# vigorbird/ORB_SLAM2_comment

Hardware: AMD Instinct MI355X
Metric: frames/sec ORB extract+match, KITTI 1241×376 @1000 feat; HBM GB/s vs peak (higher is better)
Workload: dtype u8; 1 GPU; configs[1]+[2]+[3]: a global batch of 512 synthetic 1241x376 u8 frames per step, 512 per GPU, resident in HBM as (last, cur) pairs; per step ORB extract (nFeatures=1000, 8-level pyramid) of every frame + device-resident SearchByProjection(CurrentFrame, LastFrame, th=15, mono; projection prologue included) for every pair; monocular handles: mvImagePyramid[0] on demand (orbhip_extractor_set_lazy_lev; handles_per_gpu=3, stage_gates=0, global_batch=512, nfeatures=1000, levels=8, parallelism=pair-sharded x1

## Files before the change

orb_slam2_comment_amd/csrc/orbhip_matcher.hip:

```cpp
#include "orbhip_internal.h"

#include <algorithm>
#include <climits>
#include <new>
#include <vector>

namespace orbhip {

constexpr int TH_HIGH = 100, TH_LOW = 50, HISTO_LENGTH = 30;
constexpr int GRID_ROWS = 48, GRID_COLS = 64;
constexpr int kResolveMax = 4096;
constexpr uint32_t kNoCell = 0xffffffffu;

struct DevFrame {
    int n;
    const orbhip_keypoint *keys;
    const uint8_t *desc;
    const float *u_right;
    float min_x, min_y, inv_w, inv_h;
};

struct Batch {
    const int *n_dev;
    const int *nq_dev;
// ... 30 lines not shown
        const uint32_t lo_ = (uint32_t)v, hi_ = (uint32_t)(v >> 32);                                          \
        const uint32_t ol_ = (uint32_t)__builtin_amdgcn_update_dpp((int)lo_, (int)lo_, ctrl, rmask, 0xf, false); \
        const uint32_t oh_ = (uint32_t)__builtin_amdgcn_update_dpp((int)hi_, (int)hi_, ctrl, rmask, 0xf, false); \
        const unsigned long long o_ = ((unsigned long long)oh_ << 32) | ol_;                                  \
        v = o_ < v ? o_ : v;                                                                                  \
    }
    ORBHIP_MIN64_STEP(0xB1, 0xf)
    ORBHIP_MIN64_STEP(0x4E, 0xf)
    ORBHIP_MIN64_STEP(0x141, 0xf)
    ORBHIP_MIN64_STEP(0x140, 0xf)
    ORBHIP_MIN64_STEP(0x142, 0xa)
    ORBHIP_MIN64_STEP(0x143, 0xc)
#undef ORBHIP_MIN64_STEP
    return ((unsigned long long)(uint32_t)__builtin_amdgcn_readlane((int)(v >> 32), 63) << 32) |
           (uint32_t)__builtin_amdgcn_readlane((int)(uint32_t)v, 63);
}

constexpr int kHeadMax = 8;
__device__ __forceinline__ int wave_sorted_head(unsigned long long a1, unsigned long long a2, bool more,
                                                unsigned long long (&head)[kHeadMax], bool *complete)
{
    int given = 0, hl = 0;
    bool stop = false, dry = false;
#pragma unroll
    for (int k = 0; k < kHeadMax; ++k) {
        head[k] = ~0ull;
        if (stop || dry) continue;
        const unsigned long long c = given == 0 ? a1 : (given == 1 ? a2 : ~0ull);
        const unsigned long long g = wave_min_u64(c);
        if (g == ~0ull) { dry = true; continue; }
// ... 120 lines not shown

constexpr int kGridCells = GRID_COLS * GRID_ROWS;
struct GridRec { float x, y; int octave; uint32_t key; };
__device__ __forceinline__ void grid_build_body(DevFrame F, int *__restrict__ cell_start, GridRec *__restrict__ rec,
                                                uint4 *__restrict__ rdesc, float *__restrict__ rur, const Batch &B, const int pair)
{
    __shared__ int s_cnt[kGridCells];
    __shared__ int s_scan[8];
    const int tid = threadIdx.x;
    batch_frame(F, B, pair);
    const size_t rbase = (size_t)pair * B.cap;
    cell_start += (size_t)pair * (kGridCells + 1);
    rec += rbase; rdesc += rbase * 2; rur += rbase;
    for (int c = tid; c < kGridCells; c += 256) s_cnt[c] = 0;
    __syncthreads();
    for (int j = tid; j < F.n; j += 256) {
        const orbhip_keypoint kp = F.keys[j];
        const int px = (int)roundf(__fmul_rn(__fsub_rn(kp.x, F.min_x), F.inv_w));
        const int py = (int)roundf(__fmul_rn(__fsub_rn(kp.y, F.min_y), F.inv_h));
        if (!(px < 0 || px >= GRID_COLS || py < 0 || py >= GRID_ROWS)) atomicAdd(&s_cnt[px * GRID_ROWS + py], 1);
    }
    __syncthreads();
    constexpr int PER = kGridCells / 256;
    int local[PER], sum = 0;
#pragma unroll
    for (int k = 0; k < PER; ++k) { local[k] = s_cnt[tid * PER + k]; sum += local[k]; }
    int incl = sum;
    const int lane = tid & 63, wave = tid >> 6;
    incl = wave_incl_scan_add(incl);
    if (lane == 63) s_scan[wave] = incl;
    __syncthreads();
    int base = incl - sum;
    for (int w = 0; w < wave; ++w) base += s_scan[w];
    __syncthreads();
#pragma unroll
    for (int k = 0; k < PER; ++k) { s_cnt[tid * PER + k] = base; cell_start[tid * PER + k] = base; base += local[k]; }
    if (tid == 255) cell_start[kGridCells] = base;
    __syncthreads();
    for (int j = tid; j < F.n; j += 256) {
        const orbhip_keypoint kp = F.keys[j];
        const int px = (int)roundf(__fmul_rn(__fsub_rn(kp.x, F.min_x), F.inv_w));
        const int py = (int)roundf(__fmul_rn(__fsub_rn(kp.y, F.min_y), F.inv_h));
        if (!(px < 0 || px >= GRID_COLS || py < 0 || py >= GRID_ROWS)) {
            const int cell = px * GRID_ROWS + py;
            const int pos = atomicAdd(&s_cnt[cell], 1);
            GridRec r; r.x = kp.x; r.y = kp.y; r.octave = kp.octave; r.key = ((uint32_t)cell << 20) | (uint32_t)j;
            rec[pos] = r;
            const uint4 *d = reinterpret_cast<const uint4 *>(F.desc + (size_t)j * 32);
            rdesc[2 * pos] = d[0]; rdesc[2 * pos + 1] = d[1];
            rur[pos] = F.u_right ? F.u_right[j] : -1.0f;
        }
    }
}
__global__ __launch_bounds__(256) void k_grid_build(DevFrame F, int *__restrict__ cell_start, GridRec *__restrict__ rec,
                                                    uint4 *__restrict__ rdesc, float *__restrict__ rur, Batch B)
{
    grid_build_body(F, cell_start, rec, rdesc, rur, B, (int)blockIdx.x);
}

constexpr int kCompact = 64;
__global__ __launch_bounds__(256) void k_window_search(DevFrame F, const int *__restrict__ cell_start,
                                                       const GridRec *__restrict__ rec, const uint4 *__restrict__ rdesc,
                                                       const float *__restrict__ rur,
                                                       const orbhip_query *__restrict__ q,
                                                       const uint8_t *__restrict__ qdesc,
                                                       unsigned long long *__restrict__ cand,
                                                       unsigned long long *__restrict__ ccand,
                                                       int *__restrict__ cnt, int stride, int use_ur, Batch B,
                                                       const uint8_t *__restrict__ taken, int max_dist)
{
    __shared__ unsigned long long stage[4][64];
    __shared__ int spos[4][64];
    const int lane = threadIdx.x & 63, wv = threadIdx.x >> 6;
    const int pair = blockIdx.y;
    const bool has_ur = F.u_right != nullptr;
    batch_frame(F, B, pair);
// ... 845 lines not shown
    S.lcn = lcn;
    S.lc = reinterpret_cast<uint32_t *>(base + resolve_par_bytes(n, nq, 0));
    int *p = reinterpret_cast<int *>(base);
    S.owner[0] = p; p += n; S.owner[1] = p; p += n; S.choice = p; p += nq;
    S.t_angle = reinterpret_cast<float *>(p); p += n; S.q_angle = reinterpret_cast<float *>(p); p += nq;
    S.hist = p; p += HISTO_LENGTH + 2; S.vars = p; p += 16;
    S.cur1 = reinterpret_cast<unsigned short *>(p); S.cur2 = S.cur1 + nq; p += nq;
    S.wl[0] = reinterpret_cast<unsigned short *>(p); S.wl[1] = S.wl[0] + nq; p += nq;
    S.q_cnt = p; p += nq;
    unsigned char *c = reinterpret_cast<unsigned char *>(p);
    S.t_oct = c; c += n; S.taken = c; c += n; S.q_obs = c; c += nq; S.evbin = c;
}

#ifdef ORBHIP_DEVTOOLS
__device__ unsigned int g_resolve_stats[4];
#endif
template <bool GS>
__global__ __launch_bounds__(1024) void k_resolve_par(int mode, DevFrame F, const orbhip_query *__restrict__ q, int nq,
                                                      const unsigned long long *__restrict__ cand,
                                                      const unsigned long long *__restrict__ ccand,
                                                      const int *__restrict__ cnt, int stride,
                                                      const uint8_t *__restrict__ taken_in, float nnratio,
                                                      int check_ori, int *__restrict__ out, int *__restrict__ out_n, Batch B,
                                                      int th_accept, int all_block, unsigned char *__restrict__ gstate,
                                                      size_t gstate_stride, int lcn)
{
    extern __shared__ unsigned char resolve_lds[];
    const int tid = threadIdx.x, T = blockDim.x;
    {
        const int pair = blockIdx.x;
        batch_frame(F, B, pair);
        q += (size_t)pair * B.qcap;
        cand += (size_t)pair * B.qcap * stride;
        if (ccand) ccand += (size_t)pair * B.qcap * kCompact;
        cnt += (size_t)pair * B.qcap;
        if (taken_in) taken_in += (size_t)pair * B.cap;
        out += (size_t)pair * B.cap;
        out_n += pair;
        if (B.nq_dev) nq = min(B.nq_dev[pair], B.qcap);
    }
    const int n = F.n;
    ResolveParState S;
    if (GS) resolve_par_carve(S, gstate + (size_t)blockIdx.x * gstate_stride, (size_t)n, (size_t)nq);
// ... 42 lines not shown
                    S.lc[i * (S.lcn + 1) + S.lcn] = (uint32_t)hrow[kHeadMax];
                }
                continue;
            }
            if (i != tid || !ccand) {
                const unsigned long long *l0 = ccand ? ccand + (size_t)i * kCompact : cand + (size_t)i * stride;
#pragma unroll
                for (int e = 0; e < kResolveHead; ++e) hv[e] = (e < c && e < S.lcn) ? l0[e] : ~0ull;
            }
#pragma unroll
            for (int e = 0; e < kResolveHead; ++e)
                if (e < c && e < S.lcn) S.lc[i * (S.lcn + 1) + e] = ((uint32_t)(hv[e] >> 32) << 20) | (uint32_t)(hv[e] & 0xfffffu);
        }
    }
    __syncthreads();
    auto held_by_smaller = [&](int idx, int i) -> bool {
        return S.taken[idx] || __hip_atomic_load(&holder[idx], __ATOMIC_RELAXED, __HIP_MEMORY_SCOPE_WORKGROUP) < i;
    };
    unsigned short *wl_next = nullptr;
    int *wl_count = nullptr;
    int *claim = holder;
    bool claims_rebuilt = false;
    auto pick_sorted = [&](int i, int c, unsigned long long &k1, unsigned long long &k2) {
        const unsigned long long *list = ccand ? ccand + (size_t)i * kCompact : cand + (size_t)i * stride;
        const uint32_t *lrow = S.lc + i * (S.lcn + 1);
        auto entry = [&](int e) -> unsigned long long {
            if (e >= c) return ~0ull;
            if (!GS && e < S.lcn) { const uint32_t w = lrow[e]; return ((unsigned long long)(w >> 20) << 32) | (w & 0xfffffu); }
            return list[e];
        };
// ... 139 lines not shown
                const int src = __ffsll((long long)longs) - 1;
                unsigned long long t1, t2;
                pick_unsorted_wave(__builtin_amdgcn_readlane(i, src), -__builtin_amdgcn_readlane(c, src), t1, t2);
                if (lane == src) { k1 = t1; k2 = t2; }
                longs &= longs - 1;
            }
        }
        return valid && c != 0 ? commit(i, k1, k2) : (valid ? commit(i, ~0ull, ~0ull) : false);
    };
    if (mode != 1) {
        int c_in = 5, c_out = 6, c_clr = 7, rounds = 0;
        unsigned short *w_in = S.wl[0], *w_out = S.wl[1];
        wl_next = w_out; wl_count = &S.vars[c_out];
        for (int i0 = 0; i0 < nq; i0 += T) step_group(i0 + tid, i0 + tid < nq);
        __syncthreads();
        for (;; ++rounds) {
            { unsigned short *t_ = w_in; w_in = w_out; w_out = t_; }
            { const int t_ = c_in; c_in = c_out; c_out = c_clr; c_clr = t_; }
            const int nw = S.vars[c_in];
            if (nw == 0 || rounds > 65 * nq) break;
            if (tid == 0) S.vars[c_clr] = 0;
            wl_next = w_out; wl_count = &S.vars[c_out];
            for (int k0 = 0; k0 < nw; k0 += T) step_group(k0 + tid < nw ? (int)w_in[k0 + tid] : 0, k0 + tid < nw);
            __syncthreads();
        }
        wl_next = nullptr;
        bool unobs = false;
        for (int i = tid; i < nq; i += T) unobs |= !S.q_obs[i];
        if (__syncthreads_or(unobs))
            for (int i0 = 0; i0 < nq; i0 += T) step_group(i0 + tid, i0 + tid < nq && !S.q_obs[i0 + tid]);
#ifdef ORBHIP_DEVTOOLS
        if (tid == 0) { atomicAdd(&g_resolve_stats[0], 1u); atomicAdd(&g_resolve_stats[1], (unsigned)rounds + 1); atomicMax(&g_resolve_stats[2], (unsigned)rounds + 1); }
#endif
    } else {
        int *own_cur = S.owner[0], *own_nxt = S.owner[1];
        claims_rebuilt = true;
        for (int round = 0; round <= nq + 1; ++round) {
            if (tid == 0) S.vars[0] = 0;
            for (int c = tid; c < n; c += T) own_nxt[c] = INT_MAX;
            __syncthreads();
            holder = own_cur; claim = own_nxt;
// ... 1 lines not shown
            for (int i0 = 0; i0 < nq; i0 += T) ch |= step_group(i0 + tid, i0 + tid < nq);
            if (ch) S.vars[0] = 1;
            __syncthreads();
            const int changed = S.vars[0];
            { int *t_ = own_cur; own_cur = own_nxt; own_nxt = t_; }
            __syncthreads();
            if (!changed) {
#ifdef ORBHIP_DEVTOOLS
                if (tid == 0) { atomicAdd(&g_resolve_stats[0], 1u); atomicAdd(&g_resolve_stats[1], (unsigned)round + 1); atomicMax(&g_resolve_stats[2], (unsigned)round + 1); }
#endif
                break;
            }
        }
    }
    __syncthreads();
    int *assign = S.owner[1];
    for (int c = tid; c < n; c += T) assign[c] = -1;
    __syncthreads();
    int acc_local = 0;
    const bool ori = mode == 0 && check_ori;
    for (int i0 = 0; i0 < nq; i0 += T) {
        const int i = i0 + tid;
        const int c = i < nq ? S.choice[i] : -1;
        int bin = -1;
        if (c >= 0) {
            ++acc_local;
            atomicMax(&assign[c], i);
            if (ori) {
                bin = rot_bin(S.q_angle[i], S.t_angle[c]);
                if (bin >= 0) S.evbin[i] = (unsigned char)bin;
            }
        }
        wave_hist_add(S.hist, bin);
    }
    acc_local = wave_reduce_add_i(acc_local);
    if ((tid & 63) == 0 && acc_local) atomicAdd(&S.vars[1], acc_local);
    __syncthreads();
    if (ori) {
        rank_bins_once(S.hist, S.vars + 8);
        const int ind1 = S.vars[8], ind2 = S.vars[9], ind3 = S.vars[10];
        int cull = 0;
        for (int i = tid; i < nq; i += T) {
            if (rot_culled(S.evbin[i], ind1, ind2, ind3)) {
                assign[S.choice[i]] = -1;
                ++cull;
            }
        }
        cull = wave_reduce_add_i(cull);
        if ((tid & 63) == 0 && cull) atomicAdd(&S.vars[2], cull);
        __syncthreads();
    }
    for (int c = tid; c < n; c += T) out[c] = assign[c];
    if (tid == 0) *out_n = S.vars[1] - S.vars[2];
}

struct InitState {
    int *q_cnt; float *q_angle, *t_angle;
    uint32_t *claim[2];
    int *head[2];
    unsigned short *next[2];
    unsigned char *evbin;
    int *hist, *vars;
    unsigned short *active;
    unsigned short *active_u;
    uint32_t *lc; int lcn;
};
constexpr uint32_t kNoClaim = 0xffffffffu;
__host__ __device__ constexpr size_t init_state_bytes(size_t n, size_t nq, size_t lcn)
// ... 993 lines not shown
    const float *Tcw;
    const orbhip_keypoint *keys;
    const uint8_t *desc;
    const int *n_dev;
    const float *u_right;
    const int *cell_start, *cell_items;
    const float *world, *normal, *max_dist, *min_dist;
    const uint8_t *point_desc, *flags;
    int *best_idx, *best_dist;
    orbhip_query *q;
    int cap, np, pcap;
    int sim3_form;
    int csr_by_target;
    float min_x, min_y, inv_w, inv_h;
};

template <int LPQ> __device__ __forceinline__ unsigned long long group_min_u64(unsigned long long v);
template <> __device__ __forceinline__ unsigned long long group_min_u64<64>(unsigned long long v) { return wave_min_u64(v); }
template <> __device__ __forceinline__ unsigned long long group_min_u64<8>(unsigned long long v)
{
#define ORBHIP_GMIN_STEP(ctrl)                                                                                \
    {                                                                                                         \
        const uint32_t lo_ = (uint32_t)v, hi_ = (uint32_t)(v >> 32);                                          \
        const uint32_t ol_ = (uint32_t)__builtin_amdgcn_update_dpp((int)lo_, (int)lo_, ctrl, 0xf, 0xf, false); \
        const uint32_t oh_ = (uint32_t)__builtin_amdgcn_update_dpp((int)hi_, (int)hi_, ctrl, 0xf, 0xf, false); \
        const unsigned long long o_ = ((unsigned long long)oh_ << 32) | ol_;                                  \
        v = o_ < v ? o_ : v;                                                                                  \
    }
    ORBHIP_GMIN_STEP(0xB1)
    ORBHIP_GMIN_STEP(0x4E)
    ORBHIP_GMIN_STEP(0x141)
#undef ORBHIP_GMIN_STEP
    return v;
}

template <int LPQ>
__global__ __launch_bounds__(256) void k_fuse_batch(FuseBatchArgs A, orbhip_camera cam, float th, SigmaTab sig)
{
    const int k = blockIdx.y, lane = threadIdx.x & 63;
    const int i = blockIdx.x * 256 + threadIdx.x;
    const size_t f = (size_t)A.kf_index[k], orow = (size_t)k * A.pcap;
    orbhip_query Q;
    Q.valid = 0; Q.u = 0; Q.v = 0; Q.radius = 0; Q.min_level = 0; Q.ur = 0;
    if (i < A.np) {
        KfQueryArgs P;
        P.T1 = A.Tcw + (size_t)k * 12; P.T2 = nullptr;
        P.world = A.world; P.normal = A.normal; P.max_dist = A.max_dist; P.min_dist = A.min_dist;
        P.flags = A.flags + orow; P.q = nullptr; P.n = A.np; P.mode = 0; P.double_invz = A.sim3_form;
        Q = keyframe_query(P, cam, th, i);
// ... 544 lines not shown
    __syncthreads();
    if (tid < 2) counts[(size_t)f * 2 + tid] = s_cnt[tid];
}

}

using namespace orbhip;

struct orbhip_matcher {
    int device = 0;
    hipStream_t stream = nullptr;
    hipStream_t own_stream = nullptr;
    void *buf[17] = {};
    size_t cap[17] = {};
    bool lds_attr_set = false, bow_attr_set = false;
    uint8_t *h_stage = nullptr; size_t h_stage_bytes = 0;
    uint8_t *h_out = nullptr; size_t h_out_bytes = 0;
};

static inline size_t al256(size_t b) { return (b + 255) & ~(size_t)255; }

struct Stage {
    uint8_t *h, *d;
    size_t off, cap;
    bool overrun;
    template <class T> T *take(size_t count, const T **dev)
    {
        const size_t bytes = al256(count * sizeof(T));
        if (overrun || bytes > cap - off) { overrun = true; *dev = nullptr; return nullptr; }
        *dev = reinterpret_cast<const T *>(d + off);
// ... 64 lines not shown
        m->h_out_bytes = bytes;
    }
    ORBHIP_HIP_CHECK(hipMemcpyAsync(m->h_out, d, bytes, hipMemcpyDeviceToHost, m->stream));
    ORBHIP_HIP_CHECK(hipStreamSynchronize(m->stream));
    *h = m->h_out;
    return ORBHIP_OK;
}

static int ensure_resolve_attr(orbhip_matcher *m)
{
    if (!m->lds_attr_set) {
        ORBHIP_HIP_CHECK(hipFuncSetAttribute(reinterpret_cast<const void *>(k_resolve_par<false>), hipFuncAttributeMaxDynamicSharedMemorySize,
                                             kResolveLdsBudget));
        ORBHIP_HIP_CHECK(hipFuncSetAttribute(reinterpret_cast<const void *>(k_resolve_init), hipFuncAttributeMaxDynamicSharedMemorySize,
                                             kResolveLdsBudget));
        m->lds_attr_set = true;
    }
    return ORBHIP_OK;
}

static_assert(init_state_bytes(kResolveMax, kResolveMax, 0) <= (size_t)kResolveLdsBudget, "k_resolve_init state exceeds LDS");

static int launch_resolve_par(orbhip_matcher *m, int pairs, int mode, const DevFrame &D, const orbhip_query *d_q,
                              const unsigned long long *d_cand, const unsigned long long *d_ccand, const int *d_cnt, int stride,
                              const uint8_t *d_taken, float nnratio, int check_ori, int *d_out, int *d_out_n, const Batch &B,
                              int th_accept, int all_block)
{
    if (B.cap <= kResolveMax && B.qcap <= kResolveMax) {
        const int lcn = resolve_par_bytes((size_t)B.cap, (size_t)B.qcap, kResolveHead) <= (size_t)kResolveLdsBudget ? kResolveHead : 0;
        hipLaunchKernelGGL(k_resolve_par<false>, dim3(pairs), dim3(1024), resolve_par_bytes((size_t)B.cap, (size_t)B.qcap, (size_t)lcn),
                           m->stream, mode, D, d_q, B.qcap, d_cand, d_ccand, d_cnt, stride, d_taken, nnratio, check_ori, d_out, d_out_n, B,
                           th_accept, all_block, (unsigned char *)nullptr, (size_t)0, lcn);
    } else {
        const size_t per = al256(resolve_par_bytes((size_t)B.cap, (size_t)B.qcap));
        void *p;
        int rc = scratch(m, S_STATE, per * (size_t)pairs, &p);
        if (rc) return rc;
        hipLaunchKernelGGL(k_resolve_par<true>, dim3(pairs), dim3(1024), 0, m->stream, mode, D, d_q, B.qcap, d_cand, d_ccand, d_cnt,
                           stride, d_taken, nnratio, check_ori, d_out, d_out_n, B, th_accept, all_block, (unsigned char *)p, per, 0);
    }
    return ORBHIP_OK;
}

static int launch_search(orbhip_matcher *m, int mode, int pairs, const DevFrame &D, const Batch &B, const orbhip_query *d_q,
                         const uint8_t *d_qdesc, const orbhip_keypoint *d_qkeys, const uint8_t *d_taken, float nnratio,
                         int check_ori, int th_accept, int all_block, int use_ur, int *d_out, int *d_out_n,
                         const ProjLaunch *proj = nullptr)
{
    void *p;
    int rc;
    const int stride = (B.cap + 1) & ~1;
    const size_t nql = (size_t)pairs * B.qcap;
    if ((rc = scratch(m, S_CAND, nql * stride * sizeof(unsigned long long), &p))) return rc;
    unsigned long long *d_cand = (unsigned long long *)p;
    if ((rc = scratch(m, S_CNT, nql * sizeof(int), &p))) return rc;
    int *d_cnt = (int *)p;
    if ((rc = scratch(m, S_CCAND, nql * kCompact * sizeof(unsigned long long), &p))) return rc;
    unsigned long long *d_ccand = (unsigned long long *)p;
    const size_t start_bytes = al256((size_t)pairs * (kGridCells + 1) * sizeof(int));
    const size_t nrec = (size_t)pairs * B.cap;
    if ((rc = scratch(m, S_CSR, start_bytes + al256(nrec * sizeof(GridRec)) + al256(nrec * 32) + al256(nrec * 4), &p))) return rc;
    static_assert(sizeof(GridRec) == 16, "GridRec is one dwordx4");
    int *d_start = (int *)p;
    GridRec *d_rec = (GridRec *)((uint8_t *)p + start_bytes);
    uint4 *d_rdesc = (uint4 *)((uint8_t *)d_rec + al256(nrec * sizeof(GridRec)));
    float *d_rur = (float *)((uint8_t *)d_rdesc + al256(nrec * 32));
    if ((rc = ensure_resolve_attr(m))) return rc;
    if (mode == 2) { d_taken = nullptr; use_ur = 0; }
    if (proj) {
        const int npb = (proj->P.cap + 255) / 256;
        hipLaunchKernelGGL(k_grid_build_project, dim3(pairs * (npb + 1)), dim3(256), 0, m->stream, D, d_start, d_rec, d_rdesc, d_rur, B,
                           proj->P, proj->cam, proj->th, proj->mono, npb);
    } else {
        hipLaunchKernelGGL(k_grid_build, dim3(pairs), dim3(256), 0, m->stream, D, d_start, d_rec, d_rdesc, d_rur, B);
    }
    hipLaunchKernelGGL(k_window_search, dim3((B.qcap + 3) / 4, pairs), dim3(256), 0, m->stream, D, d_start, d_rec, d_rdesc, d_rur,
                       d_q, d_qdesc, d_cand, d_ccand, d_cnt, stride, use_ur, B, d_taken, mode == 0 ? th_accept : 256);
    if (mode == 2) {
        const int lcn = init_state_bytes((size_t)B.cap, (size_t)B.qcap, kResolveHead) <= (size_t)kResolveLdsBudget ? kResolveHead : 0;
        hipLaunchKernelGGL(k_resolve_init, dim3(pairs), dim3(1024), init_state_bytes((size_t)B.cap, (size_t)B.qcap, (size_t)lcn),
                           m->stream, D, d_qkeys, B.qcap, d_cand, d_ccand, d_cnt, stride, nnratio, check_ori, d_out, d_out_n, B, lcn);
    } else if ((rc = launch_resolve_par(m, pairs, mode, D, d_q, d_cand, d_ccand, d_cnt, stride, d_taken, nnratio, check_ori, d_out,
                                        d_out_n, B, th_accept, all_block))) {
        return rc;
    }
    ORBHIP_HIP_CHECK(hipGetLastError());
    return ORBHIP_OK;
}

static int run_search(orbhip_matcher *m, int mode, const orbhip_frame_view *train, const orbhip_query *q,
                      const uint8_t *qdesc, const orbhip_keypoint *qkeys, int nq, const uint8_t *taken,
                      float nnratio, int check_ori, int32_t *out, int nout, int *nmatches, int th_accept = TH_HIGH,
// ... 37 lines not shown
        for (int k = 0; k < nqv; ++k) {
            hq[k] = q[vidx[k]];
            memcpy(hd + (size_t)k * 32, qdesc + (size_t)vidx[k] * 32, 32);
        }
    } else {
        d_q = st.put(q, (size_t)nq);
        d_qdesc = st.put(qdesc, (size_t)nq * 32);
    }
    const orbhip_keypoint *d_qkeys = qkeys ? st.put(qkeys, (size_t)nq) : nullptr;
    if ((rc = stage_commit(m, &st))) return rc;
    void *p;
    if ((rc = scratch(m, S_OUT, (size_t)(nout + 1) * sizeof(int), &p))) return rc;
    int *d_out = (int *)p;
    const Batch B = {nullptr, nullptr, train->n, nqv};
    if ((rc = launch_search(m, mode, 1, D, B, d_q, d_qdesc, d_qkeys, d_taken, nnratio, check_ori, th_accept, all_block, use_ur,
                            d_out, d_out + nout)))
        return rc;
    const uint8_t *h;
    if ((rc = read_back(m, d_out, (size_t)(nout + 1) * sizeof(int), &h))) return rc;
    memcpy(out, h, (size_t)nout * sizeof(int));
    if (compact)
        for (int i = 0; i < nout; ++i) if (out[i] >= 0) out[i] = vidx[out[i]];
    *nmatches = reinterpret_cast<const int *>(h)[nout];
    return ORBHIP_OK;
}

static void node_order(const uint32_t *node, const uint8_t *valid, int n, std::vector<int> &order)
{
    static thread_local std::vector<unsigned long long> keys;
    keys.clear();
    keys.reserve(n);
// ... 633 lines not shown

static int search_device(orbhip_matcher *m, int mode, int pairs, const void *d_kps, const void *d_desc, const void *d_n,
                         int cap, const void *d_u_right, const void *d_taken, float min_x, float min_y, float grid_inv_w,
                         float grid_inv_h, const void *d_q, const void *d_qdesc, const void *d_nq, int qcap, float nnratio,
                         int check_ori, void *d_assign, void *d_nmatches, int t0 = 0, int ts = 1, int qd0 = 0, int qds = 1,
                         const ProjLaunch *proj = nullptr)
{
    if (!m || pairs <= 0 || !d_kps || !d_desc || !d_n || !d_q || !d_qdesc || !d_nq || !d_assign || !d_nmatches || cap <= 0 || qcap <= 0)
        return ORBHIP_E_ARG;
    ORBHIP_HIP_CHECK(hipSetDevice(m->device));
    DevFrame D;
    D.n = cap; D.keys = (const orbhip_keypoint *)d_kps; D.desc = (const uint8_t *)d_desc; D.u_right = (const float *)d_u_right;
    D.min_x = min_x; D.min_y = min_y; D.inv_w = grid_inv_w; D.inv_h = grid_inv_h;
    const Batch B = {(const int *)d_n, (const int *)d_nq, cap, qcap, t0, ts, qd0, qds};
    return launch_search(m, mode, pairs, D, B, (const orbhip_query *)d_q, (const uint8_t *)d_qdesc, nullptr, (const uint8_t *)d_taken,
                         nnratio, check_ori, TH_HIGH, 0, 1, (int *)d_assign, (int *)d_nmatches, proj);
}

int orbhip_search_by_projection_frame_device(orbhip_matcher *m, int pairs, const void *d_kps, const void *d_desc,
                                             const void *d_n, int cap, const void *d_u_right, const void *d_taken,
                                             float min_x, float min_y, float grid_inv_w, float grid_inv_h,
                                             const void *d_q, const void *d_qdesc, const void *d_nq, int qcap,
                                             int check_ori, void *d_assign, void *d_nmatches)
{
    return search_device(m, 0, pairs, d_kps, d_desc, d_n, cap, d_u_right, d_taken, min_x, min_y, grid_inv_w, grid_inv_h, d_q,
                         d_qdesc, d_nq, qcap, 0.f, check_ori, d_assign, d_nmatches);
}

int orbhip_search_by_projection_points_device(orbhip_matcher *m, int pairs, const void *d_kps, const void *d_desc,
                                              const void *d_n, int cap, const void *d_u_right, const void *d_taken,
                                              float min_x, float min_y, float grid_inv_w, float grid_inv_h,
// ... 43 lines not shown
    ORBHIP_HIP_CHECK(hipSetDevice(m->device));
    int rc;
    void *p;
    if ((rc = scratch(m, S_Q, (size_t)pairs * cap * sizeof(orbhip_query), &p))) return rc;
    orbhip_query *d_q = (orbhip_query *)p;
    if ((rc = scratch(m, S_TAKEN, (size_t)pairs * sizeof(int), &p))) return rc;
    int *d_nq = (int *)p;
    const orbhip_keypoint *keys = (const orbhip_keypoint *)d_kps;
    hipLaunchKernelGGL(k_init_queries, dim3((cap + 255) / 256, pairs), dim3(256), 0, m->stream, keys, (const int *)d_n, cap,
                       f1_first, f1_step, (float *)d_prev_matched, reset_prev, (float)window_size, d_q, d_nq);
    DevFrame D;
    D.n = cap; D.keys = keys; D.desc = (const uint8_t *)d_desc; D.u_right = nullptr;
    D.min_x = min_x; D.min_y = min_y; D.inv_w = grid_inv_w; D.inv_h = grid_inv_h;
    const Batch B = {(const int *)d_n, d_nq, cap, cap, f2_first, f2_step, f1_first, f1_step};
    if ((rc = launch_search(m, 2, pairs, D, B, d_q, (const uint8_t *)d_desc, keys, nullptr, nnratio, check_ori, TH_HIGH, 0, 0,
                            (int *)d_matches12, (int *)d_nmatches)))
        return rc;
    hipLaunchKernelGGL(k_init_update_prev, dim3((cap + 255) / 256, pairs), dim3(256), 0, m->stream, keys, cap, f2_first, f2_step,
                       d_nq, (const int *)d_matches12, (float *)d_prev_matched);
    ORBHIP_HIP_CHECK(hipGetLastError());
    return ORBHIP_OK;
}

int orbhip_project_last_frame_device(orbhip_matcher *m, int pairs, const orbhip_camera *cam, const void *d_Tcw,
                                     const void *d_Tlw, const void *d_kps, const void *d_n, int cap, int last_first,
                                     int last_step, const void *d_world, const void *d_flags, float th, int mono,
                                     void *d_q, void *d_nq)
{
    if (!m || !cam || pairs <= 0 || cap <= 0 || !d_Tcw || !d_Tlw || !d_kps || !d_n || !d_world || !d_flags || !d_q ||
        cam->n_levels < 1 || cam->n_levels > ORBHIP_MAX_LEVELS)
        return ORBHIP_E_ARG;
// ... 337 lines not shown
        memcpy(min_dist, h + ((const uint8_t *)d_mn - base), sn * 4);
    }
    if (best_obs && wd) memcpy(best_obs, h + ((const uint8_t *)d_best - base), sn * 4);
    memcpy(status, h + (d_status - base), sn);
    return ORBHIP_OK;
}

#ifdef ORBHIP_DEVTOOLS
int orbhip_dev_resolve_stats(unsigned int out[4])
{
    unsigned int z[4] = {0, 0, 0, 0};
    if (hipMemcpyFromSymbol(out, HIP_SYMBOL(orbhip::g_resolve_stats), sizeof(z)) != hipSuccess) return ORBHIP_E_HIP;
    if (hipMemcpyToSymbol(HIP_SYMBOL(orbhip::g_resolve_stats), z, sizeof(z)) != hipSuccess) return ORBHIP_E_HIP;
    return ORBHIP_OK;
}
#endif

int orbhip_keyframe_queries(orbhip_matcher *m, const orbhip_camera *cam, int mode, int double_invz, const float *T1,
                            const float *T2, int n, const float *world, const float *normal, const float *max_dist,
                            const float *min_dist, const uint8_t *flags, float th, orbhip_query *q)
{
    if (!m || !cam || n < 0 || !T1 || !q || (mode != 0 && mode != 1) || (mode == 1 && !T2) || cam->n_levels < 1 ||
        cam->n_levels > ORBHIP_MAX_LEVELS)
        return ORBHIP_E_ARG;
    if (n == 0) return ORBHIP_OK;
    if (!world || !max_dist || !min_dist || !flags || (mode == 0 && !normal)) return ORBHIP_E_ARG;
    ORBHIP_HIP_CHECK(hipSetDevice(m->device));
    Stage st;
    int rc = stage_begin(m, 2 * al256(48) + 2 * al256((size_t)n * 12) + 2 * al256((size_t)n * 4) + al256((size_t)n), &st);
    if (rc) return rc;
// ... 21 lines not shown
                int n, const float *world, const float *normal, const float *max_dist, const float *min_dist,
                const uint8_t *flags, const uint8_t *point_desc, float th, const float *inv_level_sigma2, int32_t *best_idx,
                int32_t *best_dist)
{
    if (!m || !kf || n < 0 || (n > 0 && (!best_idx || !best_dist || !point_desc))) return ORBHIP_E_ARG;
    if (n == 0) return ORBHIP_OK;
    static thread_local std::vector<orbhip_query> q;
    q.resize((size_t)n);
    int rc = orbhip_keyframe_queries(m, cam, 0, sim3_form ? 1 : 0, Tcw, nullptr, n, world, normal, max_dist, min_dist, flags, th, q.data());
    if (rc) return rc;
    return orbhip_search_best_in_window(m, kf, q.data(), point_desc, n, sim3_form ? 0 : 1, inv_level_sigma2, best_idx, best_dist);
}

static int g_fuse_lanes = 8;
#ifdef ORBHIP_DEVTOOLS
int orbhip_dev_fuse_lanes(int lanes)
{
    if (lanes != 8 && lanes != 64) return ORBHIP_E_ARG;
    g_fuse_lanes = lanes;
    return ORBHIP_OK;
}
#endif

int orbhip_fuse_device(orbhip_matcher *m, int K, const void *d_kf_index, const orbhip_camera *cam, const void *d_Tcw,
                       int sim3_form, const void *d_kps, const void *d_desc, const void *d_n, int cap, const void *d_u_right,
                       const void *d_cell_start, const void *d_cell_items, int np, int pcap, const void *d_world,
                       const void *d_normal, const void *d_max_dist, const void *d_min_dist, const void *d_point_desc,
                       const void *d_flags, float th, const float *inv_level_sigma2, void *d_best_idx, void *d_best_dist,
                       void *d_q)
{
// ... 372 lines not shown
```

Baseline: 298,600 frames/s.

## Search projection windows with 16-lane groups per query and cache keypoints in grid build

Adds a k_window_search variant that assigns one 16-lane DPP row to each query instead of a full 64-lane wavefront, with group-level scan, min, ballot and rank-store helpers. A heuristic picks 16 lanes for projection searches with small thresholds and keeps 64 lanes otherwise. The aim is to cut idle lanes when windows hold few candidates, at the cost of more serial iterations per query in dense windows. Grid build also keeps up to four keypoints per thread in registers between the count and scatter passes, and devtools timing stamps are added for the resolve kernel.

```diff
diff --git a/orb_slam2_comment_amd/csrc/orbhip_matcher.hip b/orb_slam2_comment_amd/csrc/orbhip_matcher.hip
--- a/orb_slam2_comment_amd/csrc/orbhip_matcher.hip
+++ b/orb_slam2_comment_amd/csrc/orbhip_matcher.hip
@@ -68,6 +68,29 @@
 #undef ORBHIP_MIN64_STEP
     return ((unsigned long long)(uint32_t)__builtin_amdgcn_readlane((int)(v >> 32), 63) << 32) |
            (uint32_t)__builtin_amdgcn_readlane((int)(uint32_t)v, 63);
+}
+
+template <int LPQ> __device__ __forceinline__ unsigned long long group_min_u64(unsigned long long v)
+{
+    static_assert(LPQ == 8 || LPQ == 16 || LPQ == 64, "group sizes of k_fuse_batch and k_window_search");
+    if constexpr (LPQ == 64) {
+        return wave_min_u64(v);
+    } else {
+#define ORBHIP_GMIN_STEP(ctrl)                                                                                \
+    {                                                                                                         \
+        const uint32_t lo_ = (uint32_t)v, hi_ = (uint32_t)(v >> 32);                                          \
+        const uint32_t ol_ = (uint32_t)__builtin_amdgcn_update_dpp((int)lo_, (int)lo_, ctrl, 0xf, 0xf, false); \
+        const uint32_t oh_ = (uint32_t)__builtin_amdgcn_update_dpp((int)hi_, (int)hi_, ctrl, 0xf, 0xf, false); \
+        const unsigned long long o_ = ((unsigned long long)oh_ << 32) | ol_;                                  \
+        v = o_ < v ? o_ : v;                                                                                  \
+    }
+        ORBHIP_GMIN_STEP(0xB1)
+        ORBHIP_GMIN_STEP(0x4E)
+        ORBHIP_GMIN_STEP(0x141)
+        if constexpr (LPQ == 16) ORBHIP_GMIN_STEP(0x140)
+#undef ORBHIP_GMIN_STEP
+        return v;
+    }
 }
 
 constexpr int kHeadMax = 8;
@@ -218,11 +241,41 @@
     rec += rbase; rdesc += rbase * 2; rur += rbase;
     for (int c = tid; c < kGridCells; c += 256) s_cnt[c] = 0;
     __syncthreads();
-    for (int j = tid; j < F.n; j += 256) {
-        const orbhip_keypoint kp = F.keys[j];
-        const int px = (int)roundf(__fmul_rn(__fsub_rn(kp.x, F.min_x), F.inv_w));
-        const int py = (int)roundf(__fmul_rn(__fsub_rn(kp.y, F.min_y), F.inv_h));
-        if (!(px < 0 || px >= GRID_COLS || py < 0 || py >= GRID_ROWS)) atomicAdd(&s_cnt[px * GRID_ROWS + py], 1);
+    const auto cell_of = [&](float x, float y) {
+        const int px = (int)roundf(__fmul_rn(__fsub_rn(x, F.min_x), F.inv_w));
+        const int py = (int)roundf(__fmul_rn(__fsub_rn(y, F.min_y), F.inv_h));
+        return (px < 0 || px >= GRID_COLS || py < 0 || py >= GRID_ROWS) ? -1 : px * GRID_ROWS + py;
+    };
+    const auto emit = [&](int j, float x, float y, int octave, int cell) {
+        const int pos = atomicAdd(&s_cnt[cell], 1);
+        GridRec r; r.x = x; r.y = y; r.octave = octave; r.key = ((uint32_t)cell << 20) | (uint32_t)j;
+        rec[pos] = r;
+        const uint4 *d = reinterpret_cast<const uint4 *>(F.desc + (size_t)j * 32);
+        rdesc[2 * pos] = d[0]; rdesc[2 * pos + 1] = d[1];
+        rur[pos] = F.u_right ? F.u_right[j] : -1.0f;
+    };
+    constexpr int kGridKeep = 4;
+    const bool keep = F.n <= 256 * kGridKeep;
+    float kx[kGridKeep], ky[kGridKeep];
+    int ko[kGridKeep], kc[kGridKeep];
+    if (keep) {
+#pragma unroll
+        for (int k = 0; k < kGridKeep; ++k) {
+            const int j = tid + 256 * k;
+            kx[k] = ky[k] = 0.0f; ko[k] = 0; kc[k] = -1;
+            if (j < F.n) {
+                const orbhip_keypoint kp = F.keys[j];
+                kx[k] = kp.x; ky[k] = kp.y; ko[k] = kp.octave; kc[k] = cell_of(kp.x, kp.y);
+                if (kc[k] >= 0) atomicAdd(&s_cnt[kc[k]], 1);
+            }
+        }
+    } else {
+        for (int j = tid; j < F.n; j += 256) {
+            const orbhip_keypoint kp = F.keys[j];
+            const int px = (int)roundf(__fmul_rn(__fsub_rn(kp.x, F.min_x), F.inv_w));
+            const int py = (int)roundf(__fmul_rn(__fsub_rn(kp.y, F.min_y), F.inv_h));
+            if (!(px < 0 || px >= GRID_COLS || py < 0 || py >= GRID_ROWS)) atomicAdd(&s_cnt[px * GRID_ROWS + py], 1);
+        }
     }
     __syncthreads();
     constexpr int PER = kGridCells / 256;
@@ -241,18 +294,24 @@
     for (int k = 0; k < PER; ++k) { s_cnt[tid * PER + k] = base; cell_start[tid * PER + k] = base; base += local[k]; }
     if (tid == 255) cell_start[kGridCells] = base;
     __syncthreads();
-    for (int j = tid; j < F.n; j += 256) {
-        const orbhip_keypoint kp = F.keys[j];
-        const int px = (int)roundf(__fmul_rn(__fsub_rn(kp.x, F.min_x), F.inv_w));
-        const int py = (int)roundf(__fmul_rn(__fsub_rn(kp.y, F.min_y), F.inv_h));
-        if (!(px < 0 || px >= GRID_COLS || py < 0 || py >= GRID_ROWS)) {
-            const int cell = px * GRID_ROWS + py;
-            const int pos = atomicAdd(&s_cnt[cell], 1);
-            GridRec r; r.x = kp.x; r.y = kp.y; r.octave = kp.octave; r.key = ((uint32_t)cell << 20) | (uint32_t)j;
-            rec[pos] = r;
-            const uint4 *d = reinterpret_cast<const uint4 *>(F.desc + (size_t)j * 32);
-            rdesc[2 * pos] = d[0]; rdesc[2 * pos + 1] = d[1];
-            rur[pos] = F.u_right ? F.u_right[j] : -1.0f;
+    if (keep) {
+#pragma unroll
+        for (int k = 0; k < kGridKeep; ++k)
+            if (kc[k] >= 0) emit(tid + 256 * k, kx[k], ky[k], ko[k], kc[k]);
+    } else {
+        for (int j = tid; j < F.n; j += 256) {
+            const orbhip_keypoint kp = F.keys[j];
+            const int px = (int)roundf(__fmul_rn(__fsub_rn(kp.x, F.min_x), F.inv_w));
+            const int py = (int)roundf(__fmul_rn(__fsub_rn(kp.y, F.min_y), F.inv_h));
+            if (!(px < 0 || px >= GRID_COLS || py < 0 || py >= GRID_ROWS)) {
+                const int cell = px * GRID_ROWS + py;
+                const int pos = atomicAdd(&s_cnt[cell], 1);
+                GridRec r; r.x = kp.x; r.y = kp.y; r.octave = kp.octave; r.key = ((uint32_t)cell << 20) | (uint32_t)j;
+                rec[pos] = r;
+                const uint4 *d = reinterpret_cast<const uint4 *>(F.desc + (size_t)j * 32);
+                rdesc[2 * pos] = d[0]; rdesc[2 * pos + 1] = d[1];
+                rur[pos] = F.u_right ? F.u_right[j] : -1.0f;
+            }
         }
     }
 }
@@ -263,7 +322,200 @@
 }
 
 constexpr int kCompact = 64;
+template <int L> __device__ __forceinline__ int group_incl_scan_add(int v)
+{
+    static_assert(L == 16, "a group is one DPP row");
+    v += __builtin_amdgcn_update_dpp(0, v, 0x111, 0xf, 0xf, false);
+    v += __builtin_amdgcn_update_dpp(0, v, 0x112, 0xf, 0xf, false);
+    v += __builtin_amdgcn_update_dpp(0, v, 0x114, 0xf, 0xf, false);
+    v += __builtin_amdgcn_update_dpp(0, v, 0x118, 0xf, 0xf, false);
+    return v;
+}
+template <int L> __device__ __forceinline__ int group_total(int incl, int v)
+{
+    static_assert(L == 16, "a group is one DPP row");
+    (void)incl;
+    v += __builtin_amdgcn_update_dpp(0, v, 0xB1, 0xf, 0xf, false);
+    v += __builtin_amdgcn_update_dpp(0, v, 0x4E, 0xf, 0xf, false);
+    v += __builtin_amdgcn_update_dpp(0, v, 0x141, 0xf, 0xf, false);
+    v += __builtin_amdgcn_update_dpp(0, v, 0x140, 0xf, 0xf, false);
+    return v;
+}
+template <int L> __device__ __forceinline__ unsigned long long group_bits(unsigned long long bal)
+{
+    return (bal >> (threadIdx.x & 63 & ~(L - 1))) & ((1ull << L) - 1ull);
+}
+template <int L>
+__device__ __forceinline__ int group_sorted_head(unsigned long long a1, unsigned long long a2, bool more,
+                                                 unsigned long long (&head)[kHeadMax], bool *complete)
+{
+    int given = 0, hl = 0;
+    bool done = false;
+#pragma unroll
+    for (int k = 0; k < kHeadMax; ++k) {
+        head[k] = ~0ull;
+        if (!__any(!done)) continue;
+        const unsigned long long c = done ? ~0ull : (given == 0 ? a1 : (given == 1 ? a2 : ~0ull));
+        const unsigned long long g = group_min_u64<L>(c);
+        const bool got = !done && g != ~0ull;
+        if (got) { head[k] = g; hl = k + 1; }
+        const bool mine = got && c == g;
+        if (mine) ++given;
+        const bool stop = group_bits<L>(__ballot(mine && given == 2 && more)) != 0;
+        done = done || !got || stop;
+    }
+    const bool rest = (given == 0 && a1 != ~0ull) || (given <= 1 && a2 != ~0ull) || more;
+    *complete = group_bits<L>(__ballot(rest)) == 0;
+    return hl;
+}
+template <int L, int M>
+__device__ __forceinline__ void group_rank_store(const unsigned long long *__restrict__ st, const int total, const int gl,
+                                                 unsigned long long *__restrict__ row)
+{
+    unsigned long long v[M];
+    int rank[M];
+#pragma unroll
+    for (int m = 0; m < M; ++m) { v[m] = gl + m * L < total ? st[gl + m * L] : ~0ull; rank[m] = 0; }
+#pragma unroll 4
+    for (int j = 0; j < total; ++j) {
+        const unsigned long long kj = st[j];
+#pragma unroll
+        for (int m = 0; m < M; ++m) rank[m] += kj < v[m] ? 1 : 0;
+    }
+#pragma unroll
+    for (int m = 0; m < M; ++m) if (gl + m * L < total) row[rank[m]] = v[m];
+}
+template <int L>
 __global__ __launch_bounds__(256) void k_window_search(DevFrame F, const int *__restrict__ cell_start,
+                                                       const GridRec *__restrict__ rec, const uint4 *__restrict__ rdesc,
+                                                       const float *__restrict__ rur,
+                                                       const orbhip_query *__restrict__ q,
+                                                       const uint8_t *__restrict__ qdesc,
+                                                       unsigned long long *__restrict__ cand,
+                                                       unsigned long long *__restrict__ ccand,
+                                                       int *__restrict__ cnt, int stride, int use_ur, Batch B,
+                                                       const uint8_t *__restrict__ taken, int max_dist)
+{
+    static_assert(L == 16, "a group is one DPP row; the wavefront form is the specialisation below");
+    constexpr int QW = 256 / L;
+    __shared__ unsigned long long stage[QW][kCompact];
+    __shared__ int spos[QW][L];
+    const int gl = threadIdx.x & (L - 1), qw = threadIdx.x / L;
+    const int pair = blockIdx.y;
+    const bool has_ur = F.u_right != nullptr;
+    batch_frame(F, B, pair);
+    const size_t rbase = (size_t)pair * B.cap;
+    cell_start += (size_t)pair * (kGridCells + 1);
+    rec += rbase; rdesc += rbase * 2; rur += rbase;
+    q += (size_t)pair * B.qcap;
+    qdesc += (size_t)(B.qd0 + pair * B.qds) * B.qcap * 32;
+    cand += (size_t)pair * B.qcap * stride;
+    ccand += (size_t)pair * B.qcap * kCompact;
+    cnt += (size_t)pair * B.qcap;
+    if (taken) taken += (size_t)pair * B.cap;
+    const int nq = B.nq_dev ? min(B.nq_dev[pair], B.qcap) : B.qcap;
+    const int qi = blockIdx.x * QW + qw;
+    const bool inq = qi < nq;
+    orbhip_query Q = {};
+    if (inq) Q = q[qi];
+    const float x = Q.u, y = Q.v, r = Q.radius;
+    const int nMinCellX = max(0, (int)floorf(__fmul_rn(__fsub_rn(__fsub_rn(x, F.min_x), r), F.inv_w)));
+    const int nMaxCellX = min(GRID_COLS - 1, (int)ceilf(__fmul_rn(__fadd_rn(__fsub_rn(x, F.min_x), r), F.inv_w)));
+    const int nMinCellY = max(0, (int)floorf(__fmul_rn(__fsub_rn(__fsub_rn(y, F.min_y), r), F.inv_h)));
+    const int nMaxCellY = min(GRID_ROWS - 1, (int)ceilf(__fmul_rn(__fadd_rn(__fsub_rn(y, F.min_y), r), F.inv_h)));
+    const bool live = inq && Q.valid &&
+                      !(nMinCellX >= GRID_COLS || nMaxCellX < 0 || nMinCellY >= GRID_ROWS || nMaxCellY < 0 ||
+                        nMaxCellX < nMinCellX || nMaxCellY < nMinCellY);
+    if (!__any(live)) {
+        if (inq && gl == 0) cnt[qi] = 0;
+        return;
+    }
+    const bool bCheckLevels = (Q.min_level > 0) || (Q.max_level >= 0);
+    uint32_t qd[8] = {0, 0, 0, 0, 0, 0, 0, 0};
+    if (live) {
+        const uint32_t *qp = reinterpret_cast<const uint32_t *>(qdesc + (size_t)qi * 32);
+#pragma unroll
+        for (int i = 0; i < 8; ++i) qd[i] = qp[i];
+    }
+    unsigned long long *out = cand + (size_t)(inq ? qi : 0) * stride;
+    const int ncy = nMaxCellY - nMinCellY + 1;
+    int total = 0;
+    unsigned long long b1 = ~0ull, b2 = ~0ull;
+    int nb = 0;
+    const int ncol = live ? nMaxCellX - nMinCellX + 1 : 0;
+    for (int c0 = 0; __any(c0 < ncol); c0 += L) {
+        const int c = c0 + gl;
+        int start = 0, ncand = 0;
+        if (c < ncol) {
+            const int cell0 = (nMinCellX + c) * GRID_ROWS + nMinCellY;
+            start = cell_start[cell0];
+            ncand = cell_start[cell0 + ncy] - start;
+        }
+        const int incl = group_incl_scan_add<L>(ncand);
+        const int excl = incl - ncand, nrec = group_total<L>(incl, ncand);
+        for (int r0 = 0; __any(r0 < nrec); r0 += L) {
+            __builtin_amdgcn_wave_barrier();
+            for (int k = max(0, r0 - excl); k < ncand && excl + k < r0 + L; ++k) spos[qw][excl + k - r0] = start + k;
+            __builtin_amdgcn_wave_barrier();
+            bool ok = false;
+            unsigned long long key = 0;
+            if (r0 + gl < nrec) {
+                const int p = spos[qw][gl];
+                const GridRec R = rec[p];
+                const uint4 d0 = rdesc[2 * p], d1 = rdesc[2 * p + 1];
+                ok = true;
+                if (bCheckLevels) {
+                    if (R.octave < Q.min_level) ok = false;
+                    if (Q.max_level >= 0 && R.octave > Q.max_level) ok = false;
+                }
+                ok = ok && fabsf(__fsub_rn(R.x, x)) < r && fabsf(__fsub_rn(R.y, y)) < r;
+                if (ok && use_ur && has_ur) {
+                    const float ur = rur[p];
+                    if (ur > 0 && fabsf(__fsub_rn(Q.ur, ur)) > r) ok = false;
+                }
+                const int dist = __popc(qd[0] ^ d0.x) + __popc(qd[1] ^ d0.y) + __popc(qd[2] ^ d0.z) + __popc(qd[3] ^ d0.w) +
+                                 __popc(qd[4] ^ d1.x) + __popc(qd[5] ^ d1.y) + __popc(qd[6] ^ d1.z) + __popc(qd[7] ^ d1.w);
+                key = ((unsigned long long)dist << 32) | R.key;
+                ok = ok && dist <= max_dist;
+            }
+            const unsigned long long bal = group_bits<L>(__ballot(ok));
+            const int ntot = total + __popcll(bal);
+            if (ntot > kCompact && total <= kCompact)
+                for (int i = gl; i < total; i += L) out[i] = stage[qw][i];
+            if (ok) {
+                const int pos = total + __popcll(bal & ((1ull << gl) - 1ull));
+                if (ntot <= kCompact) stage[qw][pos] = key; else out[pos] = key;
+                if (!(taken && taken[key & 0xfffffu])) {
+                    if (key < b1) { b2 = b1; b1 = key; } else if (key < b2) b2 = key;
+                    ++nb;
+                }
+            }
+            total = ntot;
+        }
+    }
+    __builtin_amdgcn_wave_barrier();
+    const int ns = total <= kCompact ? total : 0;
+    unsigned long long *row = ccand + (size_t)(inq ? qi : 0) * kCompact;
+    if (__any(ns > L)) group_rank_store<L, kCompact / L>(stage[qw], ns, gl, row);
+    else group_rank_store<L, 1>(stage[qw], ns, gl, row);
+    const bool lng = total > kCompact;
+    if (__any(lng)) {
+        unsigned long long head[kHeadMax];
+        bool complete;
+        const int hl = group_sorted_head<L>(lng ? b1 : ~0ull, lng ? b2 : ~0ull, lng && nb > 2, head, &complete);
+        if (lng && gl < kHeadMax) {
+            unsigned long long v = head[0];
+#pragma unroll
+            for (int k = 1; k < kHeadMax; ++k) if (gl == k) v = head[k];
+            row[gl] = v;
+        }
+        if (lng && gl == 0) row[kHeadMax] = (unsigned long long)hl | (complete ? 0x100ull : 0ull);
+    }
+    if (inq && gl == 0) cnt[qi] = lng ? -total : total;
+}
+
+template <>
+__global__ __launch_bounds__(256) void k_window_search<64>(DevFrame F, const int *__restrict__ cell_start,
                                                        const GridRec *__restrict__ rec, const uint4 *__restrict__ rdesc,
                                                        const float *__restrict__ rur,
                                                        const orbhip_query *__restrict__ q,
@@ -1139,8 +1391,17 @@
 
 #ifdef ORBHIP_DEVTOOLS
 __device__ unsigned int g_resolve_stats[4];
+__device__ unsigned long long g_resolve_stamps[8];
 #endif
-template <bool GS>
+__device__ __forceinline__ unsigned long long resolve_stamp_now()
+{
+    unsigned long long t;
+    __builtin_amdgcn_sched_barrier(0);
+    asm volatile("s_memtime %0\n\ts_waitcnt lgkmcnt(0)" : "=s"(t) :: "memory");
+    __builtin_amdgcn_sched_barrier(0);
+    return t;
+}
+template <bool GS, bool STAMPS = false>
 __global__ __launch_bounds__(1024) void k_resolve_par(int mode, DevFrame F, const orbhip_query *__restrict__ q, int nq,
                                                       const unsigned long long *__restrict__ cand,
                                                       const unsigned long long *__restrict__ ccand,
@@ -1152,6 +1413,9 @@
 {
     extern __shared__ unsigned char resolve_lds[];
     const int tid = threadIdx.x, T = blockDim.x;
+    unsigned long long tacc[7] = {0, 0, 0, 0, 0, 0, 0}, tprev = 0;
+#define RESOLVE_STAMP(i) do { if constexpr (STAMPS) { const unsigned long long t_ = resolve_stamp_now(); tacc[i] += t_ - tprev; tprev = t_; } } while (0)
+    if constexpr (STAMPS) tprev = resolve_stamp_now();
     {
         const int pair = blockIdx.x;
         batch_frame(F, B, pair);
@@ -1224,6 +1488,7 @@
         }
     }
     __syncthreads();
+    RESOLVE_STAMP(0);
     auto held_by_smaller = [&](int idx, int i) -> bool {
         return S.taken[idx] || __hip_atomic_load(&holder[idx], __ATOMIC_RELAXED, __HIP_MEMORY_SCOPE_WORKGROUP) < i;
     };
@@ -1393,6 +1658,7 @@
         wl_next = w_out; wl_count = &S.vars[c_out];
         for (int i0 = 0; i0 < nq; i0 += T) step_group(i0 + tid, i0 + tid < nq);
         __syncthreads();
+        RESOLVE_STAMP(1);
         for (;; ++rounds) {
             { unsigned short *t_ = w_in; w_in = w_out; w_out = t_; }
             { const int t_ = c_in; c_in = c_out; c_out = c_clr; c_clr = t_; }
@@ -1404,6 +1670,7 @@
             __syncthreads();
         }
         wl_next = nullptr;
+        RESOLVE_STAMP(2);
         bool unobs = false;
         for (int i = tid; i < nq; i += T) unobs |= !S.q_obs[i];
         if (__syncthreads_or(unobs))
@@ -1435,6 +1702,7 @@
         }
     }
     __syncthreads();
+    if (mode != 1) RESOLVE_STAMP(3); else RESOLVE_STAMP(2);
     int *assign = S.owner[1];
     for (int c = tid; c < n; c += T) assign[c] = -1;
     __syncthreads();
@@ -1457,6 +1725,7 @@
     acc_local = wave_reduce_add_i(acc_local);
     if ((tid & 63) == 0 && acc_local) atomicAdd(&S.vars[1], acc_local);
     __syncthreads();
+    RESOLVE_STAMP(4);
     if (ori) {
         rank_bins_once(S.hist, S.vars + 8);
         const int ind1 = S.vars[8], ind2 = S.vars[9], ind3 = S.vars[10];
@@ -1471,8 +1740,20 @@
         if ((tid & 63) == 0 && cull) atomicAdd(&S.vars[2], cull);
         __syncthreads();
     }
+    RESOLVE_STAMP(5);
     for (int c = tid; c < n; c += T) out[c] = assign[c];
     if (tid == 0) *out_n = S.vars[1] - S.vars[2];
+    RESOLVE_STAMP(6);
+#ifdef ORBHIP_DEVTOOLS
+    if constexpr (STAMPS) {
+        if (tid == 0) {
+#pragma unroll
+            for (int i = 0; i < 7; ++i) atomicAdd(&g_resolve_stamps[i], tacc[i]);
+            atomicAdd(&g_resolve_stamps[7], 1ull);
+        }
+    }
+#endif
+#undef RESOLVE_STAMP
 }
 
 struct InitState {
@@ -2496,25 +2777,6 @@
     int csr_by_target;
     float min_x, min_y, inv_w, inv_h;
 };
-
-template <int LPQ> __device__ __forceinline__ unsigned long long group_min_u64(unsigned long long v);
-template <> __device__ __forceinline__ unsigned long long group_min_u64<64>(unsigned long long v) { return wave_min_u64(v); }
-template <> __device__ __forceinline__ unsigned long long group_min_u64<8>(unsigned long long v)
-{
-#define ORBHIP_GMIN_STEP(ctrl)                                                                                \
-    {                                                                                                         \
-        const uint32_t lo_ = (uint32_t)v, hi_ = (uint32_t)(v >> 32);                                          \
-        const uint32_t ol_ = (uint32_t)__builtin_amdgcn_update_dpp((int)lo_, (int)lo_, ctrl, 0xf, 0xf, false); \
-        const uint32_t oh_ = (uint32_t)__builtin_amdgcn_update_dpp((int)hi_, (int)hi_, ctrl, 0xf, 0xf, false); \
-        const unsigned long long o_ = ((unsigned long long)oh_ << 32) | ol_;                                  \
-        v = o_ < v ? o_ : v;                                                                                  \
-    }
-    ORBHIP_GMIN_STEP(0xB1)
-    ORBHIP_GMIN_STEP(0x4E)
-    ORBHIP_GMIN_STEP(0x141)
-#undef ORBHIP_GMIN_STEP
-    return v;
-}
 
 template <int LPQ>
 __global__ __launch_bounds__(256) void k_fuse_batch(FuseBatchArgs A, orbhip_camera cam, float th, SigmaTab sig)
@@ -3089,6 +3351,10 @@
     void *buf[17] = {};
     size_t cap[17] = {};
     bool lds_attr_set = false, bow_attr_set = false;
+#ifdef ORBHIP_DEVTOOLS
+    int window_lanes = 0;
+    bool resolve_stamps = false;
+#endif
     uint8_t *h_stage = nullptr; size_t h_stage_bytes = 0;
     uint8_t *h_out = nullptr; size_t h_out_bytes = 0;
 };
@@ -3183,6 +3449,10 @@
                                              kResolveLdsBudget));
         ORBHIP_HIP_CHECK(hipFuncSetAttribute(reinterpret_cast<const void *>(k_resolve_init), hipFuncAttributeMaxDynamicSharedMemorySize,
                                              kResolveLdsBudget));
+#ifdef ORBHIP_DEVTOOLS
+        ORBHIP_HIP_CHECK(hipFuncSetAttribute(reinterpret_cast<const void *>(k_resolve_par<false, true>),
+                                             hipFuncAttributeMaxDynamicSharedMemorySize, kResolveLdsBudget));
+#endif
         m->lds_attr_set = true;
     }
     return ORBHIP_OK;
@@ -3197,6 +3467,15 @@
 {
     if (B.cap <= kResolveMax && B.qcap <= kResolveMax) {
         const int lcn = resolve_par_bytes((size_t)B.cap, (size_t)B.qcap, kResolveHead) <= (size_t)kResolveLdsBudget ? kResolveHead : 0;
+#ifdef ORBHIP_DEVTOOLS
+        if (m->resolve_stamps) {
+            hipLaunchKernelGGL((k_resolve_par<false, true>), dim3(pairs), dim3(1024),
+                               resolve_par_bytes((size_t)B.cap, (size_t)B.qcap, (size_t)lcn), m->stream, mode, D, d_q, B.qcap, d_cand, d_ccand,
+                               d_cnt, stride, d_taken, nnratio, check_ori, d_out, d_out_n, B, th_accept, all_block,
+                               (unsigned char *)nullptr, (size_t)0, lcn);
+            return ORBHIP_OK;
+        }
+#endif
         hipLaunchKernelGGL(k_resolve_par<false>, dim3(pairs), dim3(1024), resolve_par_bytes((size_t)B.cap, (size_t)B.qcap, (size_t)lcn),
                            m->stream, mode, D, d_q, B.qcap, d_cand, d_ccand, d_cnt, stride, d_taken, nnratio, check_ori, d_out, d_out_n, B,
                            th_accept, all_block, (unsigned char *)nullptr, (size_t)0, lcn);
@@ -3211,9 +3490,18 @@
     return ORBHIP_OK;
 }
 
+constexpr float kWindowLanesTh = 20.0f;
+static int window_lanes(const orbhip_matcher *m, int mode, const ProjLaunch *proj = nullptr)
+{
+#ifdef ORBHIP_DEVTOOLS
+    if (m->window_lanes) return m->window_lanes;
+#endif
+    if (proj && proj->th > kWindowLanesTh) return 64;
+    return mode == 2 ? 64 : 16;
+}
 static int launch_search(orbhip_matcher *m, int mode, int pairs, const DevFrame &D, const Batch &B, const orbhip_query *d_q,
                          const uint8_t *d_qdesc, const orbhip_keypoint *d_qkeys, const uint8_t *d_taken, float nnratio,
-                         int check_ori, int th_accept, int all_block, int use_ur, int *d_out, int *d_out_n,
+                         int check_ori, int th_accept, int all_block, int use_ur, int *d_out, int *d_out_n, const int lanes,
                          const ProjLaunch *proj = nullptr)
 {
     void *p;
@@ -3243,8 +3531,13 @@
     } else {
         hipLaunchKernelGGL(k_grid_build, dim3(pairs), dim3(256), 0, m->stream, D, d_start, d_rec, d_rdesc, d_rur, B);
     }
-    hipLaunchKernelGGL(k_window_search, dim3((B.qcap + 3) / 4, pairs), dim3(256), 0, m->stream, D, d_start, d_rec, d_rdesc, d_rur,
-                       d_q, d_qdesc, d_cand, d_ccand, d_cnt, stride, use_ur, B, d_taken, mode == 0 ? th_accept : 256);
+    const int max_dist = mode == 0 ? th_accept : 256;
+    if (lanes == 16)
+        hipLaunchKernelGGL(k_window_search<16>, dim3((B.qcap + 15) / 16, pairs), dim3(256), 0, m->stream, D, d_start, d_rec, d_rdesc,
+                           d_rur, d_q, d_qdesc, d_cand, d_ccand, d_cnt, stride, use_ur, B, d_taken, max_dist);
+    else
+        hipLaunchKernelGGL(k_window_search<64>, dim3((B.qcap + 3) / 4, pairs), dim3(256), 0, m->stream, D, d_start, d_rec, d_rdesc,
+                           d_rur, d_q, d_qdesc, d_cand, d_ccand, d_cnt, stride, use_ur, B, d_taken, max_dist);
     if (mode == 2) {
         const int lcn = init_state_bytes((size_t)B.cap, (size_t)B.qcap, kResolveHead) <= (size_t)kResolveLdsBudget ? kResolveHead : 0;
         hipLaunchKernelGGL(k_resolve_init, dim3(pairs), dim3(1024), init_state_bytes((size_t)B.cap, (size_t)B.qcap, (size_t)lcn),
@@ -3312,7 +3605,7 @@
     int *d_out = (int *)p;
     const Batch B = {nullptr, nullptr, train->n, nqv};
     if ((rc = launch_search(m, mode, 1, D, B, d_q, d_qdesc, d_qkeys, d_taken, nnratio, check_ori, th_accept, all_block, use_ur,
-                            d_out, d_out + nout)))
+                            d_out, d_out + nout, window_lanes(m, mode))))
         return rc;
     const uint8_t *h;
     if ((rc = read_back(m, d_out, (size_t)(nout + 1) * sizeof(int), &h))) return rc;
@@ -3976,7 +4269,7 @@
     D.min_x = min_x; D.min_y = min_y; D.inv_w = grid_inv_w; D.inv_h = grid_inv_h;
     const Batch B = {(const int *)d_n, (const int *)d_nq, cap, qcap, t0, ts, qd0, qds};
     return launch_search(m, mode, pairs, D, B, (const orbhip_query *)d_q, (const uint8_t *)d_qdesc, nullptr, (const uint8_t *)d_taken,
-                         nnratio, check_ori, TH_HIGH, 0, 1, (int *)d_assign, (int *)d_nmatches, proj);
+                         nnratio, check_ori, TH_HIGH, 0, 1, (int *)d_assign, (int *)d_nmatches, window_lanes(m, mode, proj), proj);
 }
 
 int orbhip_search_by_projection_frame_device(orbhip_matcher *m, int pairs, const void *d_kps, const void *d_desc,
@@ -4050,7 +4343,7 @@
     D.min_x = min_x; D.min_y = min_y; D.inv_w = grid_inv_w; D.inv_h = grid_inv_h;
     const Batch B = {(const int *)d_n, d_nq, cap, cap, f2_first, f2_step, f1_first, f1_step};
     if ((rc = launch_search(m, 2, pairs, D, B, d_q, (const uint8_t *)d_desc, keys, nullptr, nnratio, check_ori, TH_HIGH, 0, 0,
-                            (int *)d_matches12, (int *)d_nmatches)))
+                            (int *)d_matches12, (int *)d_nmatches, window_lanes(m, 2))))
         return rc;
     hipLaunchKernelGGL(k_init_update_prev, dim3((cap + 255) / 256, pairs), dim3(256), 0, m->stream, keys, cap, f2_first, f2_step,
                        d_nq, (const int *)d_matches12, (float *)d_prev_matched);
@@ -4418,6 +4711,30 @@
     if (hipMemcpyToSymbol(HIP_SYMBOL(orbhip::g_resolve_stats), z, sizeof(z)) != hipSuccess) return ORBHIP_E_HIP;
     return ORBHIP_OK;
 }
+int orbhip_dev_window_lists(orbhip_matcher *m, int nlists, int *cnt, unsigned long long *ccand)
+{
+    if (!m || nlists < 1 || !cnt || !ccand) return ORBHIP_E_ARG;
+    const size_t n = (size_t)nlists;
+    if (m->cap[S_CNT] < n * sizeof(int) || m->cap[S_CCAND] < n * kCompact * sizeof(unsigned long long)) return ORBHIP_E_ARG;
+    ORBHIP_HIP_CHECK(hipSetDevice(m->device));
+    ORBHIP_HIP_CHECK(hipStreamSynchronize(m->stream));
+    ORBHIP_HIP_CHECK(hipMemcpy(cnt, m->buf[S_CNT], n * sizeof(int), hipMemcpyDeviceToHost));
+    ORBHIP_HIP_CHECK(hipMemcpy(ccand, m->buf[S_CCAND], n * kCompact * sizeof(unsigned long long), hipMemcpyDeviceToHost));
+    return ORBHIP_OK;
+}
+int orbhip_dev_set_resolve_stamps(orbhip_matcher *m, int on)
+{
+    if (!m) return ORBHIP_E_ARG;
+    m->resolve_stamps = on != 0;
+    return ORBHIP_OK;
+}
+int orbhip_dev_resolve_stamps(unsigned long long out[8])
+{
+    unsigned long long z[8] = {0, 0, 0, 0, 0, 0, 0, 0};
+    if (hipMemcpyFromSymbol(out, HIP_SYMBOL(orbhip::g_resolve_stamps), sizeof(z)) != hipSuccess) return ORBHIP_E_HIP;
+    if (hipMemcpyToSymbol(HIP_SYMBOL(orbhip::g_resolve_stamps), z, sizeof(z)) != hipSuccess) return ORBHIP_E_HIP;
+    return ORBHIP_OK;
+}
 #endif
 
 int orbhip_keyframe_queries(orbhip_matcher *m, const orbhip_camera *cam, int mode, int double_invz, const float *T1,
@@ -4469,6 +4786,12 @@
 
 static int g_fuse_lanes = 8;
 #ifdef ORBHIP_DEVTOOLS
+int orbhip_dev_set_window_lanes(orbhip_matcher *m, int lanes)
+{
+    if (!m || (lanes != 0 && lanes != 16 && lanes != 64)) return ORBHIP_E_ARG;
+    m->window_lanes = lanes;
+    return ORBHIP_OK;
+}
 int orbhip_dev_fuse_lanes(int lanes)
 {
     if (lanes != 8 && lanes != 64) return ORBHIP_E_ARG;
```

New measurement: 309,900 frames/s (median of 6 runs). 3.8% higher.
